# Restream/reindexer

Measured on NVIDIA H100. Metric: KNN QPS @ recall@10 (10Mx768, k=10) + HBM GB/s vs roofline, higher is better.
Workload: dtype f32

## Files before the change

### reindexer_b200/csrc/index.cu

```cuda
#include <cuda_runtime.h>

#include <cub/device/device_radix_sort.cuh>
#include <cub/device/device_scan.cuh>
#include <cub/device/device_segmented_radix_sort.cuh>
#include <cub/device/device_segmented_sort.cuh>

#include <algorithm>
#include <atomic>
#include <cstdio>
#include <cstdlib>
#include <cstring>
#include <limits>
#include <memory>
#include <mutex>
#include <new>
#include <string>
#include <unordered_map>
#include <unordered_set>
#include <vector>

#include "../../include/rxgpu.h"
#include "internal.h"
#include "../host/knn_select.h"
#include "knn_scan.cuh"
// ... 545 lines not shown
				}
				if (added) {
					tc_assign_slots<<<(added + 255) / 256, 256, 0, st>>>(kept, size, ix->shadow_slots, ix->d_slot_row, ix->d_row_slot);
					g_stats.launches += 1;
					convert(kept, size);
				}
				ix->shadow_slots = uint32_t(slots);
				ix->shadow_dead += gone;
				ix->shadow_unsorted += uint32_t(added + rewritten);
			}
		}
		if (full) {
			if (size) {
				if (int rc = sortShadowSlots(ix, st, size)) {
					return rc;
				}
				convert(0, size);
			}
			ix->shadow_slots = size;
			ix->shadow_dead = 0;
			ix->shadow_unsorted = 0;
		}
		ix->shadow_rows = size;
		ix->shadow_dirty_all = false;
		ix->shadow_dirty.clear();
		const uint32_t slots = ix->shadow_slots;
		const uint64_t padded = (uint64_t(slots) + kTcTileRows - 1) / kTcTileRows * kTcTileRows;
		RX_CUDA(cudaMemsetAsync(ix->d_rowc + slots, 0, size_t(padded - slots) * sizeof(float4), st));
		const uint32_t nblocks = uint32_t(padded / 64);
		if (nblocks) {
			tc_block_consts<<<(nblocks * 32 + 255) / 256, 256, 0, st>>>(ix->d_rowc, ix->d_slot_row, slots, nblocks,
																		   1.f - tc_l2eps(ix->dim), ix->metric, ix->d_blockc);
			g_stats.launches += 1;
		}
		RX_CUDA(cudaGetLastError());
		RX_CUDA(cudaStreamSynchronize(st));
		ix->shadow_version = ix->version;
	}
	return 0;
}

constexpr uint32_t kTcClusterDefault = 2;
constexpr uint64_t kTcClusterMinRows = 1u << 23;
uint32_t tcClusterSize(uint32_t nblocks, uint32_t ntiles, uint32_t cmax) {
	for (uint32_t c = cmax; c > 1; c /= 2) {
		const uint32_t pad = (c - nblocks % c) % c;
		if (ntiles >= 2 && pad <= 1 && pad < nblocks) {
			return c;
		}
	}
	return 1;
}

struct TcBatch {
	uint32_t nq, nqb, cluster, ngroups, nqPad, kchunks, stages, queueSlots;
	int diag;
	size_t smem;
	int resident;
	TcKernel kfn;
	CUtensorMap mapQ;
};

int tcPrepare(const rxgpu_index* ix, Workspace& ws, cudaStream_t st, const float* d_queries, uint32_t nq, uint32_t candCap, TcBatch& b) {
	if (int rc = ensureShadow(ix, st)) {
		return rc;
	}
	const uint32_t pitchQ = ix->pitch_q, kchunks = pitchQ / kTcChunkK;
	const uint32_t nqb = tcQueryBlock(nq, kchunks);
	const uint32_t ntiles = uint32_t((ix->size + kTcTileRows - 1) / kTcTileRows);
	const uint32_t nblocks = (nq + nqb - 1) / nqb;
	const uint32_t cmax = ix->tc_cluster_max ? ix->tc_cluster_max : ix->size >= kTcClusterMinRows ? kTcClusterDefault : 1u;
	const uint32_t cluster = tcClusterSize(nblocks, ntiles, cmax);
	const uint32_t ngroups = (nblocks + cluster - 1) / cluster;
	const uint32_t nqPad = ngroups * cluster * nqb;
	RX_CUDA(ws.d_qcodes.ensure(size_t(nqPad) * pitchQ));
	RX_CUDA(ws.d_qc.ensure(nqPad));
	RX_CUDA(ws.d_qf.ensure(size_t(nqPad) * pitchQ));
	RX_CUDA(ws.d_tau.ensure(nqPad));
	RX_CUDA(ws.d_cand_count.ensure(nqPad));
	RX_CUDA(ws.d_cand_rows.ensure(size_t(nqPad) * candCap));
	RX_CUDA(ws.h_cand_count.ensure(nqPad));
	tc_prepare_queries<<<(nqPad * 32 + 255) / 256, 256, 0, st>>>(d_queries, nq, nqPad, ix->dim, pitchQ, ws.d_qcodes.p, ws.d_qc.p,
																 ws.d_qf.p);
	g_stats.launches += 1;
	RX_CUDA(cudaGetLastError());
	if (int rc = makeCodeMap(&b.mapQ, ws.d_qcodes.p, pitchQ, nqPad, nqb)) {
		return rc;
	}
	b.kfn = tcKernel(nqb, cluster);
	b.stages = tc_ring_stages(nqb, kchunks, kTcSmemLimit);
	b.queueSlots = tc_queue_slots(nqb, kchunks, b.stages, kTcSmemLimit);
	b.smem = tc_smem_bytes(nqb, kchunks, b.stages) + tc_queue_bytes(b.queueSlots);
	if (b.stages == 0 || b.queueSlots == 0) {
		return fail(RXGPU_ERR_SYSTEM, "rxgpu: no room for the tensor-core filter's candidate queues");
	}
	b.diag = g_tc_diag.load();
	if (const int diag = b.diag) {
		if (nqb != 128) {
			return fail(RXGPU_ERR_PARAMS, "rxgpu: the diagnostic filter instantiations take query blocks of 128");
		}
		b.kfn = tcDiagKernel(diag, cluster);
	}
	RX_CUDA(raiseSmemCeilingOnce(b.kfn, ix->device, int(kTcSmemLimit)));
	cudaLaunchConfig_t cfg{};
	cfg.gridDim = dim3(unsigned(ix->sm_count) / cluster * cluster);
	cfg.blockDim = dim3(kTcThreads);
	cfg.dynamicSmemBytes = b.smem;
	cudaLaunchAttribute attr[1];
	attr[0].id = cudaLaunchAttributeClusterDimension;
	attr[0].val.clusterDim.x = cluster;
	attr[0].val.clusterDim.y = 1;
	attr[0].val.clusterDim.z = 1;
	cfg.attrs = attr;
	cfg.numAttrs = 1;
	b.resident = 0;
	RX_CUDA(cudaOccupancyMaxActiveClusters(&b.resident, b.kfn, &cfg));
	if (b.resident < 1) {
		return fail(RXGPU_ERR_SYSTEM, "rxgpu: tensor-core filter kernel cannot be made resident");
	}
	b.nq = nq;
	b.nqb = nqb;
	b.cluster = cluster;
	b.ngroups = ngroups;
	b.nqPad = nqPad;
	b.kchunks = kchunks;
	return 0;
}

int tcLaunch(const rxgpu_index* ix, Workspace& ws, cudaStream_t st, const TcBatch& b, uint32_t k1, uint32_t candCap, uint32_t nrows, bool fixedTau) {
	const uint32_t nq = b.nq, nqb = b.nqb, cluster = b.cluster, ngroups = b.ngroups, kchunks = b.kchunks, pitchQ = ix->pitch_q;
	const uint32_t ntiles = (nrows + kTcTileRows - 1) / kTcTileRows;
	const int resident = b.resident;
	const TcKernel kfn = b.kfn;
	const CUtensorMap mapQ = b.mapQ;
	RX_CUDA(cudaMemsetAsync(ws.d_cand_count.p, 0, size_t(b.nqPad) * 4, st));
	RX_CUDA(cudaGetLastError());
	cudaLaunchConfig_t cfg{};
	cfg.blockDim = dim3(kTcThreads);
	cfg.dynamicSmemBytes = b.smem;
	cfg.stream = st;
	cudaLaunchAttribute attr[1];
	attr[0].id = cudaLaunchAttributeClusterDimension;
	attr[0].val.clusterDim.x = cluster;
	attr[0].val.clusterDim.y = 1;
	attr[0].val.clusterDim.z = 1;
	cfg.attrs = attr;
	cfg.numAttrs = 1;
	TcArgs a{};
	a.shadow = static_cast<const unsigned char*>(ix->d_shadow);
	a.rowc = ix->d_rowc;
	a.slot_row = ix->d_slot_row;
	a.blockc = ix->d_blockc;
	a.qc = ws.d_qc.p;
	a.tau = ws.d_tau.p;
	a.ub_list = fixedTau ? nullptr : ws.d_ub_list.p;
	a.ub_lock = fixedTau ? nullptr : ws.d_ub_lock.p;
	a.init_rows = fixedTau ? UINT32_MAX : uint32_t(std::min<uint64_t>(ix->size, kTcInitRows));
	a.rows = ix->d_rows;
	a.norm_coefs = ix->metric == RXGPU_COS ? ix->d_norms : nullptr;
	a.qf = ws.d_qf.p;
	a.pitch = ix->pitch;
	a.cand_rows = ws.d_cand_rows.p;
	a.cand_count = ws.d_cand_count.p;
	a.cand_cap = candCap;
	a.n = nrows;
	a.dim = ix->dim;
	a.kchunks = kchunks;
	a.nq_total = nq;
	a.k1 = k1;
	a.metric = ix->metric;
	a.queue_slots = b.queueSlots;
	a.stages = b.stages;
	a.diag = g_tc_diag_buf;
	for (uint32_t g0 = 0; g0 < ngroups;) {
		const uint32_t groups = std::min<uint32_t>(ngroups - g0, uint32_t(resident));
		const uint32_t walkers = uint32_t(std::min<uint64_t>(uint32_t(resident) / groups, ntiles));
		cfg.gridDim = dim3(groups * walkers * cluster);
		a.q0 = g0 * cluster * nqb;
		a.groups = groups;
		cudaEvent_t e0 = nullptr, e1 = nullptr;
		if (g_profile.load(std::memory_order_relaxed)) {
			RX_CUDA(cudaEventCreate(&e0));
			RX_CUDA(cudaEventCreate(&e1));
			RX_CUDA(cudaEventRecord(e0, st));
		}
		RX_CUDA(cudaLaunchKernelEx(&cfg, kfn, mapQ, a));
		RX_CUDA(cudaGetLastError());
		if (e0) {
			RX_CUDA(cudaEventRecord(e1, st));
			g_prof_events.emplace_back(e0, e1);
		}
		g_stats.launches += 1;
		g_stats.passes += 1;
		const uint32_t served = std::min(groups * cluster * nqb, nq - a.q0);
		g_stats.algorithmic_bytes += uint64_t(nrows) * pitchQ + uint64_t(nrows) * sizeof(float4) + uint64_t(served) * pitchQ;
		g0 += groups;
	}
	g_stats.tc_cluster = cluster;
	g_stats.tc_kernel = 1 + uint32_t(b.diag);
	g_stats.query_tile = nqb * cluster;
	return 0;
}

int tcFilter(const rxgpu_index* ix, Workspace& ws, cudaStream_t st, const float* d_queries, uint32_t nq, uint32_t k1, uint32_t candCap,
			 const unsigned int* h_tau) {
	TcBatch b;
	if (int rc = tcPrepare(ix, ws, st, d_queries, nq, candCap, b)) {
		return rc;
	}
	if (h_tau) {
		RX_CUDA(cudaMemcpyAsync(ws.d_tau.p, h_tau, size_t(nq) * 4, cudaMemcpyHostToDevice, st));
	} else {
		RX_CUDA(ws.d_ub_list.ensure(size_t(b.nqPad) * kTcMaxK1));
		RX_CUDA(ws.d_ub_lock.ensure(b.nqPad));
		RX_CUDA(raiseSmemCeilingOnce(tc_init_tau, ix->device, int(tc_init_smem_bytes())));
		tc_init_tau<<<(nq + kTcInitQ - 1) / kTcInitQ, 256, tc_init_smem_bytes(), st>>>(
			ix->d_rows, ix->pitch, b.kchunks, ix->metric == RXGPU_COS ? ix->d_norms : nullptr, uint32_t(std::min<uint64_t>(ix->size, kTcInitRows)),
			ws.d_qf.p, nq, k1, ix->metric, ws.d_tau.p, ws.d_ub_list.p, ws.d_ub_lock.p);
		g_stats.launches += 1;
	}
	return tcLaunch(ix, ws, st, b, k1, candCap, ix->shadow_slots, h_tau != nullptr);
}

int rerankRange(const rxgpu_index* ix, Workspace& ws, cudaStream_t st, const float* d_queries, uint32_t nq, uint32_t nctas, const uint32_t* d_qsel,
				uint32_t cap, const float* d_radius, uint64_t* d_keys, unsigned int* d_nkeys) {
	RX_CUDA(cudaMemsetAsync(d_nkeys, 0, size_t(nq) * 4, st));
	const size_t rsmem = size_t((ix->dim + 127) / 128) * 512 + size_t(kScanWarps) * (1 + kCandBuf) * 8;
	const float* norms = ix->metric == RXGPU_COS ? ix->d_norms : nullptr;
	if (ix->metric == RXGPU_L2) {
		RX_CUDA(raiseSmemCeilingOnce(knn_rerank<true>, ix->device, kScanSmemBudget));
		knn_rerank<true><<<nctas, kScanThreads, rsmem, st>>>(ix->d_rows, ix->pitch, ix->dim, norms, d_queries, ws.d_cand_rows.p, ws.d_cand_count.p,
															  cap, 1, nullptr, d_qsel, nullptr, d_radius, d_keys, d_nkeys);
	} else {
		RX_CUDA(raiseSmemCeilingOnce(knn_rerank<false>, ix->device, kScanSmemBudget));
		knn_rerank<false><<<nctas, kScanThreads, rsmem, st>>>(ix->d_rows, ix->pitch, ix->dim, norms, d_queries, ws.d_cand_rows.p, ws.d_cand_count.p,
															   cap, 1, nullptr, d_qsel, nullptr, d_radius, d_keys, d_nkeys);
	}
	RX_CUDA(cudaGetLastError());
	g_stats.launches += 1;
	return 0;
}

int scanTopKStaged(const rxgpu_index* ix, Workspace& ws, cudaStream_t st, const float* d_queries, uint32_t nq, uint32_t k1,
				   float* d_out_dist, uint32_t* d_out_idx, uint64_t* d_out_label, uint32_t* d_out_count) {
	const uint32_t cap = stageCandCap(k1);
	const uint32_t size = uint32_t(ix->size);
	TcBatch b;
	if (int rc = tcPrepare(ix, ws, st, d_queries, nq, cap, b)) {
		return rc;
	}
	RX_CUDA(ws.d_radius.ensure(nq));
	RX_CUDA(ws.d_range_n.ensure(nq));
	RX_CUDA(ws.d_range.ensure(size_t(nq) * cap));
	RX_CUDA(ws.d_stage_status.ensure(nq));
	RX_CUDA(ws.h_stage_status.ensure(nq));
	RX_CUDA(ws.d_reranked.ensure(1));
	RX_CUDA(ws.h_reranked.ensure(1));
	RX_CUDA(cudaMemsetAsync(ws.d_reranked.p, 0, sizeof(unsigned long long), st));
	uint32_t rows = std::min(size, stageSeedRows(k1));
	if (int rc = scanTopKExact(ix, ws, st, d_queries, nq, k1, kModeTopK, 0.f, d_out_dist, d_out_idx, d_out_label, d_out_count, rows)) {
		return rc;
	}
	knn_seed_tau<<<(nq + 255) / 256, 256, 0, st>>>(d_out_dist, d_out_count, k1, nq, ws.d_tau.p, ws.d_radius.p, ws.d_stage_status.p);
	RX_CUDA(cudaGetLastError());
	g_stats.launches += 1;
	SelectArgs s{};
	s.keys = ws.d_range.p;
	s.nkeys = ws.d_range_n.p;
	s.cand_count = ws.d_cand_count.p;
	s.labels = ix->d_labels;
	s.cap = cap;
	s.k1 = k1;
	s.mode = kModeTopK;
	s.tau = ws.d_tau.p;
	s.radius = ws.d_radius.p;
	s.status = ws.d_stage_status.p;
	s.reranked = ws.d_reranked.p;
	s.out_dist = d_out_dist;
	s.out_idx = d_out_idx;
	s.out_label = d_out_label;
	s.out_count = d_out_count;
	s.neg_zero = ix->metric != RXGPU_L2;
	const uint32_t slots = ix->shadow_slots;
	uint32_t prefix = rows;
	do {
		prefix = uint32_t(std::min<uint64_t>(slots, uint64_t(prefix) * kStageRatio));
		if (int rc = tcLaunch(ix, ws, st, b, k1, cap, prefix, true)) {
			return rc;
		}
		if (int rc = rerankRange(ix, ws, st, d_queries, nq, nq, nullptr, cap, ws.d_radius.p, ws.d_range.p, ws.d_range_n.p)) {
			return rc;
		}
		s.last = prefix == slots;
		knn_select_topk<<<nq, kSelThreads, 0, st>>>(s);
		RX_CUDA(cudaGetLastError());
		g_stats.launches += 1;
	} while (prefix < slots);
	RX_CUDA(cudaMemcpyAsync(ws.h_cand_count.p, ws.d_cand_count.p, size_t(nq) * 4, cudaMemcpyDeviceToHost, st));
	RX_CUDA(cudaMemcpyAsync(ws.h_stage_status.p, ws.d_stage_status.p, size_t(nq) * 4, cudaMemcpyDeviceToHost, st));
	RX_CUDA(cudaMemcpyAsync(ws.h_reranked.p, ws.d_reranked.p, sizeof(unsigned long long), cudaMemcpyDeviceToHost, st));
	RX_CUDA(cudaStreamSynchronize(st));
	for (uint32_t q = 0; q < nq; ++q) {
		if (ws.h_stage_status.p[q]) {
			g_stats.tc_fallbacks += 1;
			ws.h_cand_count.p[q] = UINT32_MAX;
			if (int rc = scanTopKExact(ix, ws, st, d_queries + size_t(q) * ix->dim, 1, k1, kModeTopK, 0.f, d_out_dist + size_t(q) * k1,
									   d_out_idx + size_t(q) * k1, d_out_label ? d_out_label + size_t(q) * k1 : nullptr, d_out_count + q)) {
				return rc;
			}
		}
	}
	ws.tc_lists_valid = true;
	ws.tc_lists_nq = nq;
	ws.tc_lists_cap = cap;
	ws.tc_lists_version = ix->version;
	g_stats.tc_used = 1;
	g_stats.tc_candidates = *ws.h_reranked.p;
	g_stats.algorithmic_bytes += *ws.h_reranked.p * (uint64_t(ix->dim) * 4 + 4);
	return 0;
}

int scanTopKTensorCore(const rxgpu_index* ix, Workspace& ws, cudaStream_t st, const float* d_queries, uint32_t nq, uint32_t k1,
					   float* d_out_dist, uint32_t* d_out_idx, uint64_t* d_out_label, uint32_t* d_out_count) {
	const uint32_t candCap = tcCandCap(k1);
	if (int rc = tcFilter(ix, ws, st, d_queries, nq, k1, candCap, nullptr)) {
		return rc;
	}
	RX_CUDA(ws.d_lists.ensure(size_t(nq) * k1));
	const size_t rsmem = size_t((ix->dim + 127) / 128) * 512 + size_t(kScanWarps) * (k1 + kCandBuf) * 8;
	const float* norms = ix->metric == RXGPU_COS ? ix->d_norms : nullptr;
	if (ix->metric == RXGPU_L2) {
		RX_CUDA(raiseSmemCeilingOnce(knn_rerank<true>, ix->device, kScanSmemBudget));
		knn_rerank<true><<<nq, kScanThreads, rsmem, st>>>(ix->d_rows, ix->pitch, ix->dim, norms, d_queries, ws.d_cand_rows.p,
														   ws.d_cand_count.p, candCap, k1, ws.d_lists.p);
	} else {
		RX_CUDA(raiseSmemCeilingOnce(knn_rerank<false>, ix->device, kScanSmemBudget));
		knn_rerank<false><<<nq, kScanThreads, rsmem, st>>>(ix->d_rows, ix->pitch, ix->dim, norms, d_queries, ws.d_cand_rows.p,
															ws.d_cand_count.p, candCap, k1, ws.d_lists.p);
	}
	MergeArgs m{};
	m.lists = ws.d_lists.p;
	m.labels = ix->d_labels;
	m.out_dist = d_out_dist;
	m.out_idx = d_out_idx;
	m.out_label = d_out_label;
	m.out_count = d_out_count;
	m.nlists = 1;
	m.qt = nq;
	m.k1 = k1;
	m.q_offset = 0;
	m.out_stride = k1;
	m.out_offset = 0;
	m.mode = kModeTopK;
	m.neg_zero = ix->metric != RXGPU_L2;
	knn_merge_lists<<<nq, 256, 0, st>>>(m);
	RX_CUDA(cudaGetLastError());
	g_stats.launches += 2;
	RX_CUDA(cudaMemcpyAsync(ws.h_cand_count.p, ws.d_cand_count.p, size_t(nq) * 4, cudaMemcpyDeviceToHost, st));
	RX_CUDA(cudaStreamSynchronize(st));
	uint64_t cands = 0;
	for (uint32_t q = 0; q < nq; ++q) {
		cands += std::min<unsigned>(ws.h_cand_count.p[q], candCap);
		if (ws.h_cand_count.p[q] > candCap) {
			g_stats.tc_fallbacks += 1;
			if (int rc = scanTopKExact(ix, ws, st, d_queries + size_t(q) * ix->dim, 1, k1, kModeTopK, 0.f, d_out_dist + size_t(q) * k1,
									   d_out_idx + size_t(q) * k1, d_out_label ? d_out_label + size_t(q) * k1 : nullptr, d_out_count + q)) {
				return rc;
			}
		}
	}
	ws.tc_lists_valid = true;
	ws.tc_lists_nq = nq;
	ws.tc_lists_cap = candCap;
	ws.tc_lists_version = ix->version;
	g_stats.tc_used = 1;
	g_stats.tc_candidates = cands;
	g_stats.algorithmic_bytes += cands * (uint64_t(ix->dim) * 4 + 4);
	return 0;
}

}

namespace rxgpu {
int scanTopK(const rxgpu_index* ix, Workspace& ws, cudaStream_t st, const float* d_queries, uint32_t nq, uint32_t k1, int mode, float bound,
			 float* d_out_dist, uint32_t* d_out_idx, uint64_t* d_out_label, uint32_t* d_out_count) {
	if (tcEligible(ix, nq, k1, mode) && k1 > kTcMaxK1) {
		return scanTopKStaged(ix, ws, st, d_queries, nq, k1, d_out_dist, d_out_idx, d_out_label, d_out_count);
	}
	if (tcEligible(ix, nq, k1, mode)) {
		return scanTopKTensorCore(ix, ws, st, d_queries, nq, k1, d_out_dist, d_out_idx, d_out_label, d_out_count);
	}
// ... 1147 lines not shown
```

### reindexer_b200/csrc/internal.h

```cpp
#pragma once
#include <cuda_runtime.h>

#include <atomic>
#include <functional>
#include <memory>
#include <mutex>
#include <string>
#include <utility>
#include <vector>

#include "../../include/rxgpu.h"
#include "../host/flat_map.h"

namespace rxgpu {

extern thread_local std::string g_err;
extern thread_local rxgpu_search_stats g_stats;
extern thread_local std::vector<std::pair<cudaEvent_t, cudaEvent_t>> g_prof_events;
extern std::atomic<int> g_profile;

inline void collectProfile() {
	for (auto& ev : g_prof_events) {
		float ms = 0.f;
		if (cudaEventElapsedTime(&ms, ev.first, ev.second) == cudaSuccess) {
// ... 60 lines not shown
			cudaFreeHost(p);
			p = nullptr;
			n = 0;
		}
		cudaError_t e = cudaMallocHost(reinterpret_cast<void**>(&p), want * sizeof(T));
		if (e == cudaSuccess) {
			n = want;
		}
		return e;
	}
};

constexpr int kScanSmemBudget = 100 * 1024;
inline cudaError_t raiseSmemCeilingOnceImpl(const void* fn, int device, int bytes) {
	static std::mutex mtx;
	static std::vector<std::pair<const void*, int>> done;
	std::lock_guard<std::mutex> lck(mtx);
	for (const auto& d : done) {
		if (d.first == fn && d.second == device) {
			return cudaSuccess;
		}
	}
	const cudaError_t e = cudaFuncSetAttribute(fn, cudaFuncAttributeMaxDynamicSharedMemorySize, bytes);
	if (e == cudaSuccess) {
		done.emplace_back(fn, device);
	}
	return e;
}
template <typename Kernel>
inline cudaError_t raiseSmemCeilingOnce(Kernel kfn, int device, int bytes) {
	return raiseSmemCeilingOnceImpl(reinterpret_cast<const void*>(kfn), device, bytes);
}

struct Workspace {
	cudaStream_t stream = nullptr;
	DevBuf<float> d_queries;
	DevBuf<uint64_t> d_lists;
	DevBuf<uint64_t> d_floor;
	DevBuf<float> d_out_dist;
	DevBuf<uint32_t> d_out_idx;
	DevBuf<uint64_t> d_out_label;
	DevBuf<uint32_t> d_out_count;
	DevBuf<uint64_t> d_range;
	DevBuf<unsigned long long> d_range_count;
	DevBuf<float> d_radius;
	DevBuf<unsigned int> d_range_n;
	PinBuf<unsigned int> h_range_n;
	DevBuf<unsigned char> d_qcodes;
	DevBuf<float4> d_qc;
	DevBuf<float> d_qf;
	DevBuf<unsigned int> d_tau, d_cand_count, d_ub_lock;
	DevBuf<float> d_ub_list;
	DevBuf<uint32_t> d_cand_rows;
	PinBuf<unsigned int> h_cand_count;
	DevBuf<unsigned int> d_stage_status;
	PinBuf<unsigned int> h_stage_status;
	DevBuf<unsigned long long> d_reranked;
	PinBuf<unsigned long long> h_reranked;
	PinBuf<float> h_queries;
	PinBuf<float> h_out_dist;
	PinBuf<uint32_t> h_out_idx;
	PinBuf<uint64_t> h_out_label;
	PinBuf<uint32_t> h_out_count;
	PinBuf<uint64_t> h_range;
	bool tc_lists_valid = false;
	uint32_t tc_lists_nq = 0;
	uint32_t tc_lists_cap = 0;
	uint64_t tc_lists_version = 0;
	DevBuf<uint32_t> d_sel;
	DevBuf<float> d_selbound;
	DevBuf<float> d_tie_dist;
	DevBuf<uint32_t> d_tie_idx, d_tie_count;
	DevBuf<uint64_t> d_tie_label;
	~Workspace() {
		if (stream) {
			cudaStreamDestroy(stream);
		}
	}
};

}

struct rxgpu_hnsw_device;
struct rxgpu_ivf_device;
struct rxgpu_sq8_device;
namespace rxgpu {
void hnswRelease(rxgpu_hnsw_device*);
void ivfRelease(rxgpu_ivf_device*);
void sq8Release(rxgpu_sq8_device*);
}

struct rxgpu_index {
	int metric = 0;
	uint32_t dim = 0;
	uint32_t pitch = 0;
	uint64_t capacity = 0;
	uint64_t size = 0;
	int device = 0;
	uint32_t flags = 0;
	int sm_count = 132;
	uint32_t qt_override = 0;
	uint64_t version = 0;

	float* d_rows = nullptr;
	uint64_t* d_labels = nullptr;
	float* d_norms = nullptr;
// ... 162 lines not shown
```

### reindexer_b200/csrc/knn_tc.cuh

```cuda
#pragma once
#include <cuda.h>

#include <type_traits>

#include "common.cuh"
#include "knn_scan.cuh"

namespace rxgpu {

constexpr int kTcThreads = 512;
constexpr int kTcConsumers = 3;
constexpr int kTcTileRows = 128;
constexpr int kTcChunkK = 128;
constexpr int kTcStages = 12;
constexpr int kTcStagesMin = 8;
constexpr int kTcBlockBytes = 64 * kTcChunkK;
constexpr uint32_t kTcMaxNq = 128;
constexpr uint32_t kTcMaxK1 = 128;
constexpr float kTcL2Eps = 1e-5f;

struct TcArgs {
	const unsigned char* shadow;
	const float4* rowc;
	const uint32_t* slot_row;
	const float4* blockc;
	const float4* qc;
	unsigned int* tau;
	float* ub_list;
	unsigned int* ub_lock;
	uint32_t init_rows;
	const float* rows;
	const float* norm_coefs;
	const float* qf;
	uint32_t pitch;
	uint32_t* cand_rows;
	unsigned int* cand_count;
	uint32_t cand_cap;
	uint32_t n;
	uint32_t dim;
	uint32_t kchunks;
	uint32_t nq_total;
	uint32_t q0;
	uint32_t groups;
	uint32_t k1;
	int metric;
	uint32_t queue_slots;
	uint32_t stages;
	unsigned long long* diag;
};

constexpr int kTcDiagStamps = 1;
constexpr int kTcDiagNoRare = 2;
constexpr int kTcDiagNoFetch = 3;
constexpr int kTcDiagNoTest = 4;
constexpr uint32_t kTcDiagSlots = 64;
constexpr uint32_t kTcDiagWalk = 8192;
constexpr uint32_t kTcDiagMarkEvery = 64;
enum : uint32_t {
	kTcDgFull,
	kTcDgMma,
	kTcDgDrain,
	kTcDgBar1,
	kTcDgTest,
	kTcDgAppend,
	kTcDgTurn,
	kTcDgBar2,
	kTcDgTile,
	kTcDgBlocks,
	kTcDgHits,
	kTcDgQueueWait,
	kTcDgPerWg,
	kTcDgEmpty = kTcConsumers * kTcDgPerWg,
	kTcDgProd = kTcDgEmpty + 1,
	kTcDgRescored = kTcDgProd + 1,
	kTcDgInserts,
	kTcDgRescoreCycles,
};
static_assert(kTcDgRescoreCycles < kTcDiagSlots, "diagnostic counters fit their slots");

__host__ __device__ inline size_t tc_smem_bytes(uint32_t nq_block, uint32_t kchunks, uint32_t stages = kTcStages) {
	return 1024  + size_t(nq_block) * kchunks * 128 + size_t(stages) * kTcBlockBytes + 256  +
		   size_t(nq_block) * (16  + kTcConsumers * (4 + 4) ) + 64;
}

__device__ __forceinline__ uint32_t smem_u32(const void* p) { return uint32_t(__cvta_generic_to_shared(p)); }
__device__ __forceinline__ void mbar_init(uint64_t* bar, uint32_t count) {
	asm volatile("mbarrier.init.shared::cta.b64 [%0], %1;" ::"r"(smem_u32(bar)), "r"(count));
}
// ... 310 lines not shown

template <int kNq>
__device__ __forceinline__ float tc_min_thr(const float* s_thr, uint32_t ql) {
	float t = s_thr[ql];
#pragma unroll
	for (int w = 1; w < kTcConsumers; ++w) {
		t = fminf(t, s_thr[w * kNq + ql]);
	}
	return t;
}
template <int kNq, int kDiag>
__device__ __forceinline__ void tc_bookkeeper(const TcArgs& a, TcQueue* qu, const uint4* rec, uint32_t slots, uint32_t q0, const float4* s_qc,
											  float* s_thr, int lane, unsigned long long* dg) {
	[[maybe_unused]] unsigned long long n_rescored = 0, n_inserts = 0;
	[[maybe_unused]] long long rescore_cycles = 0;
	uint32_t head = 0;
	for (;;) {
		const bool fin = ld_acquire_shared(&qu->done) == 4;
		const uint32_t n = __shfl_sync(0xffffffffu, min(ld_acquire_shared(&qu->tail) - head, 32u), 0);
		if (n == 0) {
			if (__shfl_sync(0xffffffffu, fin, 0)) {
				break;
			}
			__nanosleep(256);
			continue;
		}
		bool active = uint32_t(lane) < n;
		uint32_t ql = 0, slot = 0;
		float x = 0.f;
		if (active) {
			const uint32_t t = head + lane;
			const uint4* r = rec + (t & (slots - 1));
			while (ld_acquire_shared(&r->w) != t + 1) {
			}
			ql = r->x;
			slot = r->y;
			x = __uint_as_float(r->z);
		}
		__syncwarp();
		head += n;
		if (lane == 0) {
			st_release_shared(&qu->head, head);
		}
		const uint32_t row = active ? a.slot_row[slot] : kTcDeadSlot;
		active = active && row != kTcDeadSlot;
		float d = 0.f, err = 0.f, tau = 0.f;
		if (active) {
			const float4 qc = s_qc[ql], rc = a.rowc[slot];
			const float2 de = tc_row_bound(a, x, qc, rc);
			d = de.x;
			err = de.y;
			tau = tc_min_thr<kNq>(s_thr, ql);
		}
		const bool append = active && !(d - err > tau);
		const unsigned peers = __match_any_sync(0xffffffffu, append ? ql : ~0u);
		const int leader = __ffs(peers) - 1;
		unsigned base = 0;
		if (append && lane == leader) {
			base = atomicAdd(&a.cand_count[q0 + ql], unsigned(__popc(peers)));
		}
		base = __shfl_sync(0xffffffffu, base, leader);
		if (append) {
			const unsigned pos = base + __popc(peers & ((1u << lane) - 1u));
			if (pos < a.cand_cap) {
				a.cand_rows[size_t(q0 + ql) * a.cand_cap + pos] = row;
			}
		}
		const bool rescore = append && row >= a.init_rows && d < tau;
		const unsigned todo = __ballot_sync(0xffffffffu, rescore);
		if (todo) {
			[[maybe_unused]] const long long c0 = kDiag == kTcDiagStamps ? clock64() : 0ll;
			const float dx = a.metric == kL2 ? tc_rescore<true>(a, todo, row, ql, q0, lane) : tc_rescore<false>(a, todo, row, ql, q0, lane);
			if constexpr (kDiag != 0) {
				n_rescored += __popc(todo);
				if constexpr (kDiag == kTcDiagStamps) {
					rescore_cycles += clock64() - c0;
				}
			}
			if (rescore && dx < tc_min_thr<kNq>(s_thr, ql)) {
				if constexpr (kDiag != 0) {
					++n_inserts;
				}
				const float nt = tc_bound_insert(a, q0 + ql, dx);
				for (uint32_t w = 0; w < kTcConsumers; ++w) {
					if (nt < s_thr[w * kNq + ql]) {
						s_thr[w * kNq + ql] = nt;
					}
				}
			}
		}
		__syncwarp();
	}
	if constexpr (kDiag != 0) {
		const unsigned long long ins = __reduce_add_sync(0xffffffffu, uint32_t(n_inserts));
		if (lane == 0) {
			atomicAdd(&dg[kTcDgRescored], n_rescored);
			atomicAdd(&dg[kTcDgInserts], ins);
			atomicAdd(&dg[kTcDgRescoreCycles], (unsigned long long)rescore_cycles);
		}
	}
}

template <int kNq, int kCluster, int kDiag = 0>
__global__ void __launch_bounds__(kTcThreads, 1)
	knn_tc_filter(const __grid_constant__ CUtensorMap map_queries, const __grid_constant__ TcArgs a) {
	static_assert(kNq % 32 == 0 && kNq <= int(kTcMaxNq), "query block");
	static_assert(kCluster == 1 || kCluster == 2 || kCluster == 4, "a stage is split in 1, 2 or 4 equal copies");
	constexpr bool kStamp = kDiag == kTcDiagStamps;
	auto clk = [] {
		if constexpr (kStamp) {
			return clock64();
		} else {
			return 0ll;
		}
	};
	unsigned long long* dg = kDiag ? a.diag + size_t(blockIdx.x) * kTcDiagSlots : nullptr;
	extern __shared__ unsigned char smem_raw[];
	unsigned char* base = smem_raw + ((1024u - (smem_u32(smem_raw) & 1023u)) & 1023u);
// ... 281 lines not shown
				dt[kTcDgBar1] += s3 - s2;
				dt[kTcDgTest] += s4 - s3;
				dt[kTcDgAppend] += s5 - s4;
				dt[kTcDgBar2] += s6 - s5;
				dt[kTcDgTile] += s6 - s0;
				dt[kTcDgBlocks] += 1;
				const uint32_t h = __reduce_add_sync(0xffffffffu, nh);
				if (lane == 0 && h && walk < kTcDiagWalk) {
					atomicAdd(&a.diag[size_t(gridDim.x) * kTcDiagSlots + walk], (unsigned long long)h);
				}
			}
		}
		__syncwarp();
		if (lane == 0) {
			__threadfence_block();
			atomicAdd(&qu->done, 1u);
		}
		if constexpr (kDiag != 0) {
			const uint32_t h = __reduce_add_sync(0xffffffffu, uint32_t(nhits));
			const uint32_t x = __reduce_xor_sync(0xffffffffu, sink);
			if (lane == 0) {
				atomicAdd(&dg[wg * kTcDgPerWg + kTcDgHits], (unsigned long long)h);
				if constexpr (kDiag == kTcDiagNoTest) {
					atomicXor(&dg[wg * kTcDgPerWg + kTcDgTurn], (unsigned long long)x);
				}
				if constexpr (kStamp) {
					dt[kTcDgMma] -= dt[kTcDgFull] + dt[kTcDgTurn];
					for (uint32_t i = 0; i < kTcDgPerWg; ++i) {
						if (i != kTcDgHits) {
							atomicAdd(&dg[wg * kTcDgPerWg + i], (unsigned long long)dt[i]);
						}
					}
				}
			}
		}
	}
	__syncthreads();
	if constexpr (kStamp) {
		if (threadIdx.x < kTcConsumers) {
			dg[threadIdx.x * kTcDgPerWg + kTcDgQueueWait] = s_queue[threadIdx.x].full_waits;
		}
	}
	if constexpr (kCluster > 1) {
		cluster_sync_all();
	}
}

template <bool kIsL2>
__global__ void __launch_bounds__(kScanThreads) knn_rerank(const float* rows, uint32_t pitch, uint32_t dim, const float* norm_coefs,
															const float* queries, const uint32_t* cand_rows, const unsigned int* cand_count,
															uint32_t cand_cap, uint32_t k1, uint64_t* lists ,
															const uint32_t* qsel = nullptr, const float* tie_bound = nullptr,
															const float* radius = nullptr, uint64_t* range_keys = nullptr,
															unsigned int* range_count = nullptr) {
	extern __shared__ __align__(16) unsigned char smem_raw[];
	const int lane = threadIdx.x & 31, warp = threadIdx.x >> 5;
	const uint32_t q = qsel ? qsel[blockIdx.x] : blockIdx.x;
	const bool tie = tie_bound != nullptr;
	const bool range = radius != nullptr;
	const float rad = range ? radius[q] : 0.f;
	const float bound = tie ? tie_bound[blockIdx.x] : 0.f;
	const uint32_t nch = (dim + 127u) / 128u, dp4 = nch * 32u, pitch4 = pitch >> 2;
	const uint32_t m = k1 + kCandBuf;
	float4* sq4 = reinterpret_cast<float4*>(smem_raw);
	uint64_t* skeys = reinterpret_cast<uint64_t*>(smem_raw + size_t(dp4) * 16);
	{
		float* sq = reinterpret_cast<float*>(sq4);
		for (uint32_t i = threadIdx.x; i < dp4 * 4; i += blockDim.x) {
			sq[i] = i < dim ? queries[size_t(q) * dim + i] : 0.f;
		}
		for (uint32_t i = threadIdx.x; i < kScanWarps * m; i += blockDim.x) {
			skeys[i] = kKeyNone;
		}
	}
	__syncthreads();
	uint64_t* wkeys = skeys + size_t(warp) * m;
	uint64_t thr = kKeyNone;
	uint32_t cnt = 0;
	const uint32_t ncand = min(cand_count[q], cand_cap);
	const float4* rows4 = reinterpret_cast<const float4*>(rows);
	const uint32_t* my = cand_rows + size_t(q) * cand_cap;
	for (uint32_t i = warp; i < ncand; i += kScanWarps) {
		const uint32_t row = my[i];
		const float dist = row_dist_warp<kIsL2>(rows4, pitch4, nch, row, sq4, norm_coefs, lane);
		if (range) {
			if (lane == 0 && dist < rad) {
				range_keys[size_t(q) * cand_cap + atomicAdd(&range_count[q], 1u)] = make_key(dist, row);
			}
			continue;
		}
		const uint64_t key = !tie ? make_key(dist, row) : (dist <= bound ? ((uint64_t(row) << 32) | float_ord(dist)) : kKeyNone);
		if (key < thr) {
			if (lane == 0) {
				wkeys[k1 + cnt] = key;
			}
			++cnt;
			__syncwarp();
			if (cnt == kCandBuf) {
				warp_select(wkeys, k1 + cnt, k1, lane);
				thr = wkeys[k1 - 1];
				cnt = 0;
			}
		}
	}
	if (range) {
		return;
	}
	if (cnt) {
		warp_select(wkeys, k1 + cnt, k1, lane);
	}
	__syncthreads();
	if (warp == 0) {
		uint64_t last = 0;
		bool first = true;
		for (uint32_t r = 0; r < k1; ++r) {
			uint64_t best = kKeyNone;
			for (uint32_t i = lane; i < kScanWarps * k1; i += 32) {
				const uint32_t w = i / k1, j = i - w * k1;
				const uint64_t kx = skeys[size_t(w) * m + j];
				if ((first || kx > last) && kx < best) {
					best = kx;
				}
			}
#pragma unroll
			for (int off = 16; off > 0; off >>= 1) {
				const uint64_t ok = __shfl_xor_sync(0xffffffffu, best, off);
				best = ok < best ? ok : best;
			}
			if (lane == 0) {
				lists[size_t(blockIdx.x) * k1 + r] = best;
			}
			last = best;
			first = false;
		}
	}
}

constexpr uint32_t kTcStagedMaxK1 = 1024;
constexpr int kSelThreads = 512;
constexpr uint32_t kSelSort = 4096;

__global__ void knn_seed_tau(const float* seed_dist, const uint32_t* seed_count, uint32_t k1, uint32_t nq, unsigned int* tau, float* radius,
							 unsigned int* status) {
	const uint32_t q = blockIdx.x * blockDim.x + threadIdx.x;
	if (q >= nq) {
		return;
	}
	const float t = seed_count[q] >= k1 ? seed_dist[size_t(q) * k1 + k1 - 1] : NAN;
	const bool ok = isfinite(t);
	tau[q] = float_ord(ok ? t : -INFINITY);
	radius[q] = ok ? nextafterf(t, INFINITY) : -INFINITY;
	status[q] = ok ? 0u : 1u;
}

// ... 266 lines not shown
		return;
	}
	float u_lo = INFINITY, u_hi = 0.f, rho_hi = 0.f, nu_hi = 0.f, w_lo = INFINITY, w_hi = 0.f;
	bool live = false, pass_all = false;
	for (uint32_t i = 0; i < 2; ++i) {
		const uint32_t slot = blk * 64 + 2 * lane + i;
		if (slot >= nslots || slot_row[slot] == kTcDeadSlot) {
			continue;
		}
		live = true;
		const float4 rc = rowc[slot];
		const double S = double(rc.x) * double(rc.w);
		if (!(S > 0.0) || !isfinite(S) || !isfinite(rc.y) || !isfinite(rc.z)) {
			pass_all = true;
			continue;
		}
		const float u0 = __double2float_rd(__ddiv_rd(1.0, S)), u1 = __double2float_ru(__ddiv_ru(1.0, S));
		const float rho = __double2float_ru(__ddiv_ru(double(rc.y), double(rc.x)));
		const float nu = __double2float_ru(__ddiv_ru(double(rc.z), double(rc.x)));
		float w0 = 0.f, w1 = 0.f;
		if (metric == kL2) {
			const double nn = double(rc.z) * double(rc.z);
			w0 = __double2float_rd(__ddiv_rd(__dmul_rd(nn, double(one_minus_eps)), 2.0 * S));
			w1 = __double2float_ru(__ddiv_ru(__dmul_ru(nn, double(one_minus_eps)), 2.0 * S));
		}
		if (!isfinite(u1) || !isfinite(rho) || !isfinite(nu) || !isfinite(w1) || u0 == 0.f) {
			pass_all = true;
			continue;
		}
		u_lo = fminf(u_lo, u0);
		u_hi = fmaxf(u_hi, u1);
		rho_hi = fmaxf(rho_hi, rho);
		nu_hi = fmaxf(nu_hi, nu);
		w_lo = fminf(w_lo, w0);
		w_hi = fmaxf(w_hi, w1);
	}
	for (int off = 16; off > 0; off >>= 1) {
		u_lo = fminf(u_lo, __shfl_xor_sync(0xffffffffu, u_lo, off));
		u_hi = fmaxf(u_hi, __shfl_xor_sync(0xffffffffu, u_hi, off));
		rho_hi = fmaxf(rho_hi, __shfl_xor_sync(0xffffffffu, rho_hi, off));
		nu_hi = fmaxf(nu_hi, __shfl_xor_sync(0xffffffffu, nu_hi, off));
		w_lo = fminf(w_lo, __shfl_xor_sync(0xffffffffu, w_lo, off));
		w_hi = fmaxf(w_hi, __shfl_xor_sync(0xffffffffu, w_hi, off));
	}
	live = __any_sync(0xffffffffu, live);
	pass_all = __any_sync(0xffffffffu, pass_all);
	if (lane == 0) {
		const float flag = pass_all ? 1.f : live ? 0.f : -1.f;
		blockc[2 * blk] = flag == 0.f ? make_float4(u_lo, u_hi, rho_hi, nu_hi) : make_float4(0.f, 0.f, 0.f, 0.f);
		blockc[2 * blk + 1] = flag == 0.f ? make_float4(w_lo, w_hi, flag, 0.f) : make_float4(0.f, 0.f, flag, 0.f);
	}
}

constexpr int kTcInitQ = 4;
constexpr uint32_t kTcInitRows = 4096;
__host__ __device__ inline size_t tc_init_smem_bytes() { return size_t(kTcInitQ) * kTcInitRows * sizeof(float); }
__global__ void __launch_bounds__(256) tc_init_tau(const float* rows, uint32_t pitch, uint32_t kchunks, const float* norm_coefs, uint32_t nrows,
												   const float* qf, uint32_t nq, uint32_t k1, int metric, unsigned int* tau, float* ub_list,
												   unsigned int* ub_lock) {
	extern __shared__ __align__(16) float s_d[];
	const uint32_t q0 = blockIdx.x * kTcInitQ;
	const uint32_t lane = threadIdx.x & 31, warp = threadIdx.x >> 5;
	const float4* rows4 = reinterpret_cast<const float4*>(rows);
	const float4* q4[kTcInitQ];
#pragma unroll
	for (int qi = 0; qi < kTcInitQ; ++qi) {
		q4[qi] = reinterpret_cast<const float4*>(qf) + size_t(q0 + qi < nq ? q0 + qi : q0) * kchunks * 32u;
	}
	constexpr uint32_t kRows = 4;
	for (uint32_t r0 = warp * kRows; r0 < kTcInitRows; r0 += 8 * kRows) {
		float dist[kRows][kTcInitQ];
		if (r0 < nrows) {
			uint32_t rr[kRows];
			const float4* qp[kRows][kTcInitQ];
#pragma unroll
			for (uint32_t x = 0; x < kRows; ++x) {
				rr[x] = min(r0 + x, nrows - 1);
#pragma unroll
				for (int qi = 0; qi < kTcInitQ; ++qi) {
					qp[x][qi] = q4[qi];
				}
			}
			if (metric == kL2) {
				row_dists_warp<true, kRows, kTcInitQ>(rows4, pitch / 4, kchunks, rr, qp, nullptr, lane, dist);
			} else {
				row_dists_warp<false, kRows, kTcInitQ>(rows4, pitch / 4, kchunks, rr, qp, norm_coefs, lane, dist);
			}
		}
#pragma unroll
		for (uint32_t x = 0; x < kRows; ++x) {
#pragma unroll
			for (int qi = 0; qi < kTcInitQ; ++qi) {
				if (lane == uint32_t(qi)) {
					const uint32_t r = r0 + x;
					s_d[qi * kTcInitRows + r] = r < nrows ? dist[x][qi] : INFINITY;
				}
			}
		}
	}
	__syncthreads();
	if (warp < kTcInitQ && q0 + warp < nq) {
		const uint32_t q = q0 + warp;
		float* d = s_d + warp * kTcInitRows;
		float last = INFINITY;
		for (uint32_t round = 0; round < kTcMaxK1; ++round) {
			float best = INFINITY;
			uint32_t at = lane;
			if (round < k1) {
				for (uint32_t j = lane; j < kTcInitRows; j += 32) {
					const float y = d[j];
					if (y < best) {
						best = y;
						at = j;
					}
				}
				for (int off = 16; off > 0; off >>= 1) {
					const float ob = __shfl_xor_sync(0xffffffffu, best, off);
					const uint32_t oa = __shfl_xor_sync(0xffffffffu, at, off);
					if (ob < best || (ob == best && oa < at)) {
						best = ob;
						at = oa;
					}
				}
				if (lane == 0) {
					d[at] = INFINITY;
				}
				__syncwarp();
				last = best;
			}
			if (lane == 0) {
				ub_list[size_t(q) * kTcMaxK1 + round] = round < k1 ? best : -INFINITY;
			}
		}
		if (lane == 0) {
			tau[q] = float_ord(last);
			ub_lock[q] = 0;
		}
	}
}

__global__ void tc_prepare_queries(const float* queries, uint32_t nq, uint32_t nq_pad, uint32_t dim, uint32_t pitch, unsigned char* codes,
								   float4* qc, float* qf) {
	const uint32_t q = (blockIdx.x * blockDim.x + threadIdx.x) / 32;
	const int lane = threadIdx.x & 31;
	if (q >= nq_pad) {
		return;
	}
	for (uint32_t c = lane; c < pitch; c += 32) {
		qf[size_t(q) * pitch + c] = q < nq && c < dim ? queries[size_t(q) * dim + c] : 0.f;
	}
	unsigned char* out = codes + size_t(q) * pitch;
	const float3 srn = tc_quantize(queries + size_t(q) * dim, q < nq ? dim : 0u, pitch, lane,
								   [&](uint32_t c, uint32_t code4) { *reinterpret_cast<uint32_t*>(out + c) = code4; });
	if (lane == 0 && q < nq) {
		qc[q] = make_float4(srn.x, srn.y, srn.z, srn.x > 0.f ? 1.f / srn.x : 1.f);
	}
}

}
```

Before: 77100.

## Split tau seeding into parallel distance and select kernels; prune candidates by lower bound

The single tau-initialisation kernel becomes two launches. The first computes seed distances for 16 queries per block with queries staged in shared memory, and splits the seed rows across blocks to fill the SMs. The second runs the per-query top-k1 select from a global seed buffer. The filter now stores each candidate's lower bound (d - err), and rerank compacts away candidates whose bound exceeds the final tau before computing exact distances. This cuts init latency and rerank work, at the cost of an extra float store per candidate, block-level syncs in rerank, and a new buffer reused for seeding.

New measurement: 80250, median of 6. +4.1%, better.

```diff
diff --git a/reindexer_b200/csrc/index.cu b/reindexer_b200/csrc/index.cu
--- a/reindexer_b200/csrc/index.cu
+++ b/reindexer_b200/csrc/index.cu
@@ -621,6 +621,33 @@
 	return 1;
 }
 
+int tcSeed(const rxgpu_index* ix, Workspace& ws, cudaStream_t st, uint32_t nq, uint32_t kchunks, uint32_t k1, uint32_t candCap) {
+	const uint32_t nrows = uint32_t(std::min<uint64_t>(ix->size, kTcInitRows));
+	float* seed = ws.d_cand_lb.p;
+	if (candCap < kTcInitRows) {
+		return fail(RXGPU_ERR_SYSTEM, "rxgpu: candidate lists shorter than the filter's seed");
+	}
+	const uint32_t ntiles = (nq + kTcInitQ - 1) / kTcInitQ, step = tc_init_step(ix->metric == RXGPU_L2);
+	const uint32_t nslices = std::max(1u, std::min((nrows + step - 1) / step, uint32_t(ix->sm_count) / ntiles));
+	const uint32_t slice = (nrows + nslices * step - 1) / (nslices * step) * step;
+	const dim3 grid(ntiles, (nrows + slice - 1) / slice);
+	const size_t smem = tc_init_dists_smem_bytes(kchunks);
+	const float* norms = ix->metric == RXGPU_COS ? ix->d_norms : nullptr;
+	if (ix->metric == RXGPU_L2) {
+		RX_CUDA(raiseSmemCeilingOnce(tc_init_tau_dists<true>, ix->device, int(tc_init_dists_smem_bytes(kTcInitMaxChunks))));
+		tc_init_tau_dists<true><<<grid, kTcInitThreads, smem, st>>>(ix->d_rows, ix->pitch, kchunks, norms, nrows, slice, ws.d_qf.p, nq, seed);
+	} else {
+		RX_CUDA(raiseSmemCeilingOnce(tc_init_tau_dists<false>, ix->device, int(tc_init_dists_smem_bytes(kTcInitMaxChunks))));
+		tc_init_tau_dists<false><<<grid, kTcInitThreads, smem, st>>>(ix->d_rows, ix->pitch, kchunks, norms, nrows, slice, ws.d_qf.p, nq, seed);
+	}
+	RX_CUDA(raiseSmemCeilingOnce(tc_init_tau_select, ix->device, int(tc_init_select_smem_bytes())));
+	tc_init_tau_select<<<(nq + kTcInitSelQ - 1) / kTcInitSelQ, kTcInitSelQ * 32, tc_init_select_smem_bytes(), st>>>(
+		seed, nrows, nq, k1, ws.d_tau.p, ws.d_ub_list.p, ws.d_ub_lock.p);
+	RX_CUDA(cudaGetLastError());
+	g_stats.launches += 2;
+	return 0;
+}
+
 struct TcBatch {
 	uint32_t nq, nqb, cluster, ngroups, nqPad, kchunks, stages, queueSlots;
 	int diag;
@@ -630,7 +657,8 @@
 	CUtensorMap mapQ;
 };
 
-int tcPrepare(const rxgpu_index* ix, Workspace& ws, cudaStream_t st, const float* d_queries, uint32_t nq, uint32_t candCap, TcBatch& b) {
+int tcPrepare(const rxgpu_index* ix, Workspace& ws, cudaStream_t st, const float* d_queries, uint32_t nq, uint32_t candCap, uint32_t seedK1,
+			  TcBatch& b) {
 	if (int rc = ensureShadow(ix, st)) {
 		return rc;
 	}
@@ -653,6 +681,14 @@
 																 ws.d_qf.p);
 	g_stats.launches += 1;
 	RX_CUDA(cudaGetLastError());
+	if (seedK1) {
+		RX_CUDA(ws.d_ub_list.ensure(size_t(nqPad) * kTcMaxK1));
+		RX_CUDA(ws.d_ub_lock.ensure(nqPad));
+		RX_CUDA(ws.d_cand_lb.ensure(size_t(nqPad) * candCap));
+		if (int rc = tcSeed(ix, ws, st, nq, kchunks, seedK1, candCap)) {
+			return rc;
+		}
+	}
 	if (int rc = makeCodeMap(&b.mapQ, ws.d_qcodes.p, pitchQ, nqPad, nqb)) {
 		return rc;
 	}
@@ -730,6 +766,7 @@
 	a.qf = ws.d_qf.p;
 	a.pitch = ix->pitch;
 	a.cand_rows = ws.d_cand_rows.p;
+	a.cand_lb = fixedTau ? nullptr : ws.d_cand_lb.p;
 	a.cand_count = ws.d_cand_count.p;
 	a.cand_cap = candCap;
 	a.n = nrows;
@@ -774,19 +811,11 @@
 int tcFilter(const rxgpu_index* ix, Workspace& ws, cudaStream_t st, const float* d_queries, uint32_t nq, uint32_t k1, uint32_t candCap,
 			 const unsigned int* h_tau) {
 	TcBatch b;
-	if (int rc = tcPrepare(ix, ws, st, d_queries, nq, candCap, b)) {
+	if (int rc = tcPrepare(ix, ws, st, d_queries, nq, candCap, h_tau ? 0u : k1, b)) {
 		return rc;
 	}
 	if (h_tau) {
 		RX_CUDA(cudaMemcpyAsync(ws.d_tau.p, h_tau, size_t(nq) * 4, cudaMemcpyHostToDevice, st));
-	} else {
-		RX_CUDA(ws.d_ub_list.ensure(size_t(b.nqPad) * kTcMaxK1));
-		RX_CUDA(ws.d_ub_lock.ensure(b.nqPad));
-		RX_CUDA(raiseSmemCeilingOnce(tc_init_tau, ix->device, int(tc_init_smem_bytes())));
-		tc_init_tau<<<(nq + kTcInitQ - 1) / kTcInitQ, 256, tc_init_smem_bytes(), st>>>(
-			ix->d_rows, ix->pitch, b.kchunks, ix->metric == RXGPU_COS ? ix->d_norms : nullptr, uint32_t(std::min<uint64_t>(ix->size, kTcInitRows)),
-			ws.d_qf.p, nq, k1, ix->metric, ws.d_tau.p, ws.d_ub_list.p, ws.d_ub_lock.p);
-		g_stats.launches += 1;
 	}
 	return tcLaunch(ix, ws, st, b, k1, candCap, ix->shadow_slots, h_tau != nullptr);
 }
@@ -815,7 +844,7 @@
 	const uint32_t cap = stageCandCap(k1);
 	const uint32_t size = uint32_t(ix->size);
 	TcBatch b;
-	if (int rc = tcPrepare(ix, ws, st, d_queries, nq, cap, b)) {
+	if (int rc = tcPrepare(ix, ws, st, d_queries, nq, cap, 0, b)) {
 		return rc;
 	}
 	RX_CUDA(ws.d_radius.ensure(nq));
@@ -901,11 +930,13 @@
 	if (ix->metric == RXGPU_L2) {
 		RX_CUDA(raiseSmemCeilingOnce(knn_rerank<true>, ix->device, kScanSmemBudget));
 		knn_rerank<true><<<nq, kScanThreads, rsmem, st>>>(ix->d_rows, ix->pitch, ix->dim, norms, d_queries, ws.d_cand_rows.p,
-														   ws.d_cand_count.p, candCap, k1, ws.d_lists.p);
+														   ws.d_cand_count.p, candCap, k1, ws.d_lists.p, nullptr, nullptr, nullptr,
+														   nullptr, nullptr, ws.d_cand_lb.p, ws.d_tau.p);
 	} else {
 		RX_CUDA(raiseSmemCeilingOnce(knn_rerank<false>, ix->device, kScanSmemBudget));
 		knn_rerank<false><<<nq, kScanThreads, rsmem, st>>>(ix->d_rows, ix->pitch, ix->dim, norms, d_queries, ws.d_cand_rows.p,
-															ws.d_cand_count.p, candCap, k1, ws.d_lists.p);
+															ws.d_cand_count.p, candCap, k1, ws.d_lists.p, nullptr, nullptr, nullptr,
+															nullptr, nullptr, ws.d_cand_lb.p, ws.d_tau.p);
 	}
 	MergeArgs m{};
 	m.lists = ws.d_lists.p;
diff --git a/reindexer_b200/csrc/internal.h b/reindexer_b200/csrc/internal.h
--- a/reindexer_b200/csrc/internal.h
+++ b/reindexer_b200/csrc/internal.h
@@ -136,6 +136,7 @@
 	DevBuf<unsigned int> d_tau, d_cand_count, d_ub_lock;
 	DevBuf<float> d_ub_list;
 	DevBuf<uint32_t> d_cand_rows;
+	DevBuf<float> d_cand_lb;
 	PinBuf<unsigned int> h_cand_count;
 	DevBuf<unsigned int> d_stage_status;
 	PinBuf<unsigned int> h_stage_status;
diff --git a/reindexer_b200/csrc/knn_tc.cuh b/reindexer_b200/csrc/knn_tc.cuh
--- a/reindexer_b200/csrc/knn_tc.cuh
+++ b/reindexer_b200/csrc/knn_tc.cuh
@@ -34,6 +34,7 @@
 	const float* qf;
 	uint32_t pitch;
 	uint32_t* cand_rows;
+	float* cand_lb;
 	unsigned int* cand_count;
 	uint32_t cand_cap;
 	uint32_t n;
@@ -450,7 +451,8 @@
 			err = de.y;
 			tau = tc_min_thr<kNq>(s_thr, ql);
 		}
-		const bool append = active && !(d - err > tau);
+		const float lb = d - err;
+		const bool append = active && !(lb > tau);
 		const unsigned peers = __match_any_sync(0xffffffffu, append ? ql : ~0u);
 		const int leader = __ffs(peers) - 1;
 		unsigned base = 0;
@@ -462,6 +464,9 @@
 			const unsigned pos = base + __popc(peers & ((1u << lane) - 1u));
 			if (pos < a.cand_cap) {
 				a.cand_rows[size_t(q0 + ql) * a.cand_cap + pos] = row;
+				if (a.ub_list) {
+					a.cand_lb[size_t(q0 + ql) * a.cand_cap + pos] = lb;
+				}
 			}
 		}
 		const bool rescore = append && row >= a.init_rows && d < tau;
@@ -849,8 +854,11 @@
 															uint32_t cand_cap, uint32_t k1, uint64_t* lists ,
 															const uint32_t* qsel = nullptr, const float* tie_bound = nullptr,
 															const float* radius = nullptr, uint64_t* range_keys = nullptr,
-															unsigned int* range_count = nullptr) {
+															unsigned int* range_count = nullptr, const float* cand_lb = nullptr,
+															const unsigned int* tau = nullptr) {
 	extern __shared__ __align__(16) unsigned char smem_raw[];
+	__shared__ uint32_t s_rows[kScanThreads];
+	__shared__ uint32_t s_kept[kScanWarps];
 	const int lane = threadIdx.x & 31, warp = threadIdx.x >> 5;
 	const uint32_t q = qsel ? qsel[blockIdx.x] : blockIdx.x;
 	const bool tie = tie_bound != nullptr;
@@ -877,26 +885,47 @@
 	const uint32_t ncand = min(cand_count[q], cand_cap);
 	const float4* rows4 = reinterpret_cast<const float4*>(rows);
 	const uint32_t* my = cand_rows + size_t(q) * cand_cap;
-	for (uint32_t i = warp; i < ncand; i += kScanWarps) {
-		const uint32_t row = my[i];
-		const float dist = row_dist_warp<kIsL2>(rows4, pitch4, nch, row, sq4, norm_coefs, lane);
-		if (range) {
-			if (lane == 0 && dist < rad) {
-				range_keys[size_t(q) * cand_cap + atomicAdd(&range_count[q], 1u)] = make_key(dist, row);
-			}
-			continue;
-		}
-		const uint64_t key = !tie ? make_key(dist, row) : (dist <= bound ? ((uint64_t(row) << 32) | float_ord(dist)) : kKeyNone);
-		if (key < thr) {
-			if (lane == 0) {
-				wkeys[k1 + cnt] = key;
-			}
-			++cnt;
-			__syncwarp();
-			if (cnt == kCandBuf) {
-				warp_select(wkeys, k1 + cnt, k1, lane);
-				thr = wkeys[k1 - 1];
-				cnt = 0;
+	const float* my_lb = cand_lb ? cand_lb + size_t(q) * cand_cap : nullptr;
+	const float tau_final = cand_lb ? ord_float(tau[q]) : 0.f;
+	for (uint32_t base = 0; base < ncand; base += kScanThreads) {
+		const uint32_t e = base + threadIdx.x;
+		const bool keep = e < ncand && (my_lb == nullptr || !(my_lb[e] > tau_final));
+		const unsigned ballot = __ballot_sync(0xffffffffu, keep);
+		if (lane == 0) {
+			s_kept[warp] = __popc(ballot);
+		}
+		__syncthreads();
+		uint32_t at = 0, nkept = 0;
+#pragma unroll
+		for (int w = 0; w < kScanWarps; ++w) {
+			at += w < warp ? s_kept[w] : 0u;
+			nkept += s_kept[w];
+		}
+		if (keep) {
+			s_rows[at + __popc(ballot & ((1u << lane) - 1u))] = my[e];
+		}
+		__syncthreads();
+		for (uint32_t i = warp; i < nkept; i += kScanWarps) {
+			const uint32_t row = s_rows[i];
+			const float dist = row_dist_warp<kIsL2>(rows4, pitch4, nch, row, sq4, norm_coefs, lane);
+			if (range) {
+				if (lane == 0 && dist < rad) {
+					range_keys[size_t(q) * cand_cap + atomicAdd(&range_count[q], 1u)] = make_key(dist, row);
+				}
+				continue;
+			}
+			const uint64_t key = !tie ? make_key(dist, row) : (dist <= bound ? ((uint64_t(row) << 32) | float_ord(dist)) : kKeyNone);
+			if (key < thr) {
+				if (lane == 0) {
+					wkeys[k1 + cnt] = key;
+				}
+				++cnt;
+				__syncwarp();
+				if (cnt == kCandBuf) {
+					warp_select(wkeys, k1 + cnt, k1, lane);
+					thr = wkeys[k1 - 1];
+					cnt = 0;
+				}
 			}
 		}
 	}
@@ -1269,90 +1298,108 @@
 	}
 }
 
-constexpr int kTcInitQ = 4;
 constexpr uint32_t kTcInitRows = 4096;
-__host__ __device__ inline size_t tc_init_smem_bytes() { return size_t(kTcInitQ) * kTcInitRows * sizeof(float); }
-__global__ void __launch_bounds__(256) tc_init_tau(const float* rows, uint32_t pitch, uint32_t kchunks, const float* norm_coefs, uint32_t nrows,
-												   const float* qf, uint32_t nq, uint32_t k1, int metric, unsigned int* tau, float* ub_list,
-												   unsigned int* ub_lock) {
+constexpr int kTcInitThreads = 256;
+constexpr int kTcInitQ = 16;
+constexpr uint32_t kTcInitMaxChunks = 16;
+__host__ __device__ constexpr int tc_init_rows_per_warp(bool l2) { return l2 ? 4 : 8; }
+__host__ __device__ constexpr uint32_t tc_init_step(bool l2) { return kTcInitThreads / 32 * tc_init_rows_per_warp(l2); }
+constexpr int kTcInitSelQ = 4;
+__host__ __device__ inline size_t tc_init_dists_smem_bytes(uint32_t kchunks) { return size_t(kTcInitQ) * kchunks * 512u; }
+__host__ __device__ inline size_t tc_init_select_smem_bytes() { return size_t(kTcInitSelQ) * kTcInitRows * sizeof(float); }
+
+template <bool kIsL2>
+__global__ void __launch_bounds__(kTcInitThreads, 1) tc_init_tau_dists(const float* rows, uint32_t pitch, uint32_t kchunks, const float* norm_coefs,
+																	   uint32_t nrows, uint32_t slice_rows, const float* qf, uint32_t nq,
+																	   float* seed ) {
+	constexpr int R = tc_init_rows_per_warp(kIsL2);
+	extern __shared__ __align__(16) float4 s_q[];
+	const uint32_t lane = threadIdx.x & 31, warp = threadIdx.x >> 5;
+	const uint32_t qt = blockIdx.x * kTcInitQ, qstride = kchunks * 32u;
+	const float4* qf4 = reinterpret_cast<const float4*>(qf) + size_t(qt) * qstride;
+	for (uint32_t i = threadIdx.x; i < kTcInitQ * qstride; i += kTcInitThreads) {
+		s_q[i] = qt + i / qstride < nq ? qf4[i] : make_float4(0.f, 0.f, 0.f, 0.f);
+	}
+	__syncthreads();
+	const float4* rows4 = reinterpret_cast<const float4*>(rows);
+	const uint32_t end = min(nrows, (blockIdx.y + 1) * slice_rows);
+	for (uint32_t r0 = blockIdx.y * slice_rows + warp * R; r0 < end; r0 += tc_init_step(kIsL2)) {
+		uint32_t rr[R];
+		const float4* qp[R][kTcInitQ];
+#pragma unroll
+		for (int x = 0; x < R; ++x) {
+			rr[x] = min(r0 + x, nrows - 1);
+#pragma unroll
+			for (int qi = 0; qi < kTcInitQ; ++qi) {
+				qp[x][qi] = s_q + qi * qstride;
+			}
+		}
+		float dist[R][kTcInitQ];
+		row_dists_warp<kIsL2, R, kTcInitQ>(rows4, pitch / 4, kchunks, rr, qp, kIsL2 ? nullptr : norm_coefs, lane, dist);
+		float4 mine = make_float4(0.f, 0.f, 0.f, 0.f);
+#pragma unroll
+		for (int qi = 0; qi < kTcInitQ; ++qi) {
+#pragma unroll
+			for (int h = 0; h < R / 4; ++h) {
+				if (lane == uint32_t(qi + kTcInitQ * h)) {
+					mine = make_float4(dist[4 * h][qi], dist[4 * h + 1][qi], dist[4 * h + 2][qi], dist[4 * h + 3][qi]);
+				}
+			}
+		}
+		const uint32_t ql = lane % kTcInitQ;
+		if (lane / kTcInitQ < uint32_t(R / 4) && qt + ql < nq) {
+			*reinterpret_cast<float4*>(seed + size_t(qt + ql) * kTcInitRows + r0 + (lane / kTcInitQ) * 4) = mine;
+		}
+	}
+}
+static_assert(kTcInitQ == 16, "tc_init_tau_dists stores a query's distances from lanes q and q + 16");
+
+__global__ void __launch_bounds__(kTcInitSelQ * 32) tc_init_tau_select(const float* seed, uint32_t nrows, uint32_t nq, uint32_t k1,
+																		unsigned int* tau, float* ub_list, unsigned int* ub_lock) {
 	extern __shared__ __align__(16) float s_d[];
-	const uint32_t q0 = blockIdx.x * kTcInitQ;
 	const uint32_t lane = threadIdx.x & 31, warp = threadIdx.x >> 5;
-	const float4* rows4 = reinterpret_cast<const float4*>(rows);
-	const float4* q4[kTcInitQ];
-#pragma unroll
-	for (int qi = 0; qi < kTcInitQ; ++qi) {
-		q4[qi] = reinterpret_cast<const float4*>(qf) + size_t(q0 + qi < nq ? q0 + qi : q0) * kchunks * 32u;
-	}
-	constexpr uint32_t kRows = 4;
-	for (uint32_t r0 = warp * kRows; r0 < kTcInitRows; r0 += 8 * kRows) {
-		float dist[kRows][kTcInitQ];
-		if (r0 < nrows) {
-			uint32_t rr[kRows];
-			const float4* qp[kRows][kTcInitQ];
-#pragma unroll
-			for (uint32_t x = 0; x < kRows; ++x) {
-				rr[x] = min(r0 + x, nrows - 1);
-#pragma unroll
-				for (int qi = 0; qi < kTcInitQ; ++qi) {
-					qp[x][qi] = q4[qi];
-				}
-			}
-			if (metric == kL2) {
-				row_dists_warp<true, kRows, kTcInitQ>(rows4, pitch / 4, kchunks, rr, qp, nullptr, lane, dist);
-			} else {
-				row_dists_warp<false, kRows, kTcInitQ>(rows4, pitch / 4, kchunks, rr, qp, norm_coefs, lane, dist);
-			}
-		}
-#pragma unroll
-		for (uint32_t x = 0; x < kRows; ++x) {
-#pragma unroll
-			for (int qi = 0; qi < kTcInitQ; ++qi) {
-				if (lane == uint32_t(qi)) {
-					const uint32_t r = r0 + x;
-					s_d[qi * kTcInitRows + r] = r < nrows ? dist[x][qi] : INFINITY;
-				}
-			}
-		}
-	}
-	__syncthreads();
-	if (warp < kTcInitQ && q0 + warp < nq) {
-		const uint32_t q = q0 + warp;
-		float* d = s_d + warp * kTcInitRows;
-		float last = INFINITY;
-		for (uint32_t round = 0; round < kTcMaxK1; ++round) {
-			float best = INFINITY;
-			uint32_t at = lane;
-			if (round < k1) {
-				for (uint32_t j = lane; j < kTcInitRows; j += 32) {
-					const float y = d[j];
-					if (y < best) {
-						best = y;
-						at = j;
-					}
-				}
-				for (int off = 16; off > 0; off >>= 1) {
-					const float ob = __shfl_xor_sync(0xffffffffu, best, off);
-					const uint32_t oa = __shfl_xor_sync(0xffffffffu, at, off);
-					if (ob < best || (ob == best && oa < at)) {
-						best = ob;
-						at = oa;
-					}
-				}
-				if (lane == 0) {
-					d[at] = INFINITY;
-				}
-				__syncwarp();
-				last = best;
+	const uint32_t q = blockIdx.x * kTcInitSelQ + warp;
+	if (q >= nq) {
+		return;
+	}
+	float* d = s_d + warp * kTcInitRows;
+	for (uint32_t j = lane; j < kTcInitRows; j += 32) {
+		d[j] = j < nrows ? seed[size_t(q) * kTcInitRows + j] : INFINITY;
+	}
+	__syncwarp();
+	float last = INFINITY;
+	for (uint32_t round = 0; round < kTcMaxK1; ++round) {
+		float best = INFINITY;
+		uint32_t at = lane;
+		if (round < k1) {
+			for (uint32_t j = lane; j < kTcInitRows; j += 32) {
+				const float y = d[j];
+				if (y < best) {
+					best = y;
+					at = j;
+				}
+			}
+			for (int off = 16; off > 0; off >>= 1) {
+				const float ob = __shfl_xor_sync(0xffffffffu, best, off);
+				const uint32_t oa = __shfl_xor_sync(0xffffffffu, at, off);
+				if (ob < best || (ob == best && oa < at)) {
+					best = ob;
+					at = oa;
+				}
 			}
 			if (lane == 0) {
-				ub_list[size_t(q) * kTcMaxK1 + round] = round < k1 ? best : -INFINITY;
-			}
+				d[at] = INFINITY;
+			}
+			__syncwarp();
+			last = best;
 		}
 		if (lane == 0) {
-			tau[q] = float_ord(last);
-			ub_lock[q] = 0;
-		}
+			ub_list[size_t(q) * kTcMaxK1 + round] = round < k1 ? best : -INFINITY;
+		}
+	}
+	if (lane == 0) {
+		tau[q] = float_ord(last);
+		ub_lock[q] = 0;
 	}
 }
 
```
